# dart-icra/DART-Dual-Arm-Non-Prehensile-Manipulation

Measured on AMD Instinct MI355X. Metric: MPC solves/sec (horizon N=20, batch=18 objects) at 1/2/4/8 GPUs; max |u−u_ref|, higher is better.
Workload: dtype f64

## Files before the change

### dart-dual-arm-non-prehensile-manipulation_amd/csrc/pmpc_ipm.hip

```cpp
#if DART_WG == 2
#define dartmpc dartmpc_wg2
#endif
#include <hip/hip_runtime.h>
#include <stdint.h>
#include <stdlib.h>

#include "pmpc_ipm.h"
#include "pmpc_model.h"
#include "pmpc_resto.h"
#include "stamps.h"
#include "wave.h"

namespace dartmpc {

#ifdef DART_STAMPS
#ifndef PMPC_SEQ
__device__ unsigned long long g_stamp[32];
#define STAMP_FLUSH(b) STAMP_FLUSH32_TO(g_stamp, b)
#else
__device__ unsigned long long g_stamp_seq[32];
#define STAMP_FLUSH(b) STAMP_FLUSH32_TO(g_stamp_seq, b)
#endif
#else
#define STAMP_FLUSH(b) STAMP_FLUSH_TO(g_stamp, b)
// ... 119 lines not shown
    constexpr bool short2 = SHORT2 && !ONEROW;
    const double f11 = c.f11, a12k = c.a12k, a22k = c.a22k, ai12k = c.ai12k, ai22k = c.ai22k, a22i = c.a22i;
    const double uonf = c.uonf, A11k = c.A11k, A12k = c.A12k, A22k = c.A22k;
    (void)lane; (void)ai12k; (void)ai22k; (void)a22i; (void)uonf;
    const double X11d = lsm ? 1.0 : qp2 + delta, X22d = lsm ? 1.0 : qv2 + delta;
    double Quu[NAX], Rt[NAX];
#pragma unroll
    for (int j = 0; j < NAX; ++j) {
        P11[j] = X11d; P12[j] = 0.0; P22[j] = X22d;
        Rt[j] = (lsm ? 1.0 : Rt0[j]) + delta;
    }
    use_scan = false;
    if constexpr (NAX == 1 && QSCAN) {
        const double ratio = fmax(E11[0] * X11d, E22[0] * X22d);
        use_scan = !wany(uon && !(Rt[0] > 0.0 && ratio <= 2.0 * Rt[0]));
    }
    if (PM_EXPECT(use_scan, 1)) {
        const double iR = uon ? frcp(Rt[0]) : 0.0;
        const double G11 = be1[0] * be1[0] * iR, G12 = be1[0] * be2[0] * iR, G22 = be2[0] * be2[0] * iR;
        const double g11 = G11 + ai12k * G12, g12 = G12 + ai12k * G22, g21 = ai22k * G12, g22 = ai22k * G22;
        const double X11k = X11d * uonf, X22k = X22d * uonf;
        double T[16] = {1.0, ai12k, g11, g12,
                        0.0, ai22k, g21, g22,
                        X11k, X11k * ai12k, fma(X11k, g11, 1.0), X11k * g12,
                        0.0, X22k * ai22k, fma(X22k, g21, a12k), fma(X22k, g22, a22i)};
        mat4_scan_level<0x101, true>(T);
        mat4_scan_level<0x102>(T);
        mat4_scan_level<0x104>(T);
        if constexpr (!short2 && !one_row) mat4_scan_level<0x108>(T);
        double W[8] = {fma(T[2], X11d, T[0]), fma(T[3], X22d, T[1]), fma(T[6], X11d, T[4]),
                       fma(T[7], X22d, T[5]), fma(T[10], X11d, T[8]), fma(T[11], X22d, T[9]),
                       fma(T[14], X11d, T[12]), fma(T[15], X22d, T[13])};
        if constexpr (short2 || one_row) {
            double F[8];
            if constexpr (short2) {
#pragma unroll
            for (int e = 0; e < 8; ++e) F[e] = half_bcast_c<16>(W[e]);
            if ((lane & 16) == 0) {
#pragma unroll
                for (int i = 0; i < 4; ++i)
#pragma unroll
                    for (int jj = 0; jj < 2; ++jj)
                        W[2 * i + jj] = fma(T[4 * i], F[jj], fma(T[4 * i + 1], F[2 + jj],
                                            fma(T[4 * i + 2], F[4 + jj], T[4 * i + 3] * F[6 + jj])));
            }
            }
#pragma unroll
            for (int e = 0; e < 8; ++e) F[e] = dpp_fill<0x108, 0xf, 0>(W[e]);
            if ((lane & 24) == 0) {
#pragma unroll
                for (int i = 0; i < 4; ++i)
#pragma unroll
                    for (int jj = 0; jj < 2; ++jj)
                        W[2 * i + jj] = fma(T[4 * i], F[jj], fma(T[4 * i + 1], F[2 + jj],
                                            fma(T[4 * i + 2], F[4 + jj], T[4 * i + 3] * F[6 + jj])));
            }
        } else if constexpr (!one_row && kWaves == 1) {
            double F[8];
#pragma unroll
            for (int e = 0; e < 8; ++e) F[e] = half_bcast_c<16>(W[e]);
            if ((lane & 16) == 0) {
#pragma unroll
                for (int i = 0; i < 4; ++i)
#pragma unroll
                    for (int jj = 0; jj < 2; ++jj)
                        W[2 * i + jj] = fma(T[4 * i], F[jj], fma(T[4 * i + 1], F[2 + jj],
                                            fma(T[4 * i + 2], F[4 + jj], T[4 * i + 3] * F[6 + jj])));
            }
        }
        double pnx[3] = {0.0, 0.0, 0.0};
        if constexpr (kWaves == 2) {
            auto rows = [&]() {
                double F[8];
#pragma unroll
                for (int e = 0; e < 8; ++e) F[e] = half_bcast_c<16>(W[e]);
                if ((lane & 16) == 0) {
#pragma unroll
                    for (int i = 0; i < 4; ++i)
#pragma unroll
                        for (int jj = 0; jj < 2; ++jj)
                            W[2 * i + jj] = fma(T[4 * i], F[jj], fma(T[4 * i + 1], F[2 + jj],
                                                fma(T[4 * i + 2], F[4 + jj], T[4 * i + 3] * F[6 + jj])));
                }
            };
            double v[3] = {0.0, 0.0, 0.0}, pn[3];
            if (wave_idx() == 1) {
                rows();
                const double idet = frcp(fma(W[0], W[3], -W[1] * W[2]));
                v[0] = fma(W[4], W[3], -W[5] * W[2]) * idet;
                v[1] = 0.5 * (fma(W[5], W[0], -W[4] * W[1]) * idet + fma(W[6], W[3], -W[7] * W[2]) * idet);
                v[2] = fma(W[7], W[0], -W[6] * W[1]) * idet;
            }
            pm_pass<0>(1, 0, v, pn);
            pnx[0] = pn[0]; pnx[1] = pn[1]; pnx[2] = pn[2];
            if (wave_idx() == 0) {
#pragma unroll
                for (int i = 0; i < 4; ++i) {
                    W[2 * i] = fma(T[4 * i + 3], pn[1], fma(T[4 * i + 2], pn[0], T[4 * i]));
                    W[2 * i + 1] = fma(T[4 * i + 3], pn[2], fma(T[4 * i + 2], pn[1], T[4 * i + 1]));
                }
                rows();
            }
        }
        const double U11 = W[0], U12 = W[1], U21 = W[2], U22 = W[3];
        const double Y11 = W[4], Y12 = W[5], Y21 = W[6], Y22 = W[7];
        const double idet = frcp(fma(U11, U22, -U12 * U21));
        const double q11 = fma(Y11, U22, -Y12 * U21) * idet, q12 = fma(Y12, U11, -Y11 * U12) * idet;
        const double q21 = fma(Y21, U22, -Y22 * U21) * idet, q22 = fma(Y22, U11, -Y21 * U12) * idet;
        P11[0] = q11; P12[0] = 0.5 * (q12 + q21); P22[0] = q22;
        double n11, n12, n22;
        if constexpr (kWaves == 1) {
            n11 = from_next(P11[0]); n12 = from_next(P12[0]); n22 = from_next(P22[0]);
        } else {
            n11 = dpp<kWaveShl1>(P11[0]); n12 = dpp<kWaveShl1>(P12[0]); n22 = dpp<kWaveShl1>(P22[0]);
            if (wave_idx() == 0 && (lane & 31) == 31) { n11 = pnx[0]; n12 = pnx[1]; n22 = pnx[2]; }
        }
        const double e1 = be1[0], e2 = be2[0];
        const double Q = fma(E11[0], n11, fma(E12[0], n12, fma(E22[0], n22, Rt[0])));
        const double PB1 = fma(n11, e1, n12 * e2), PB2 = fma(n12, e1, n22 * e2);
        const double U1 = PB1, U2 = fma(PB1, a12k, PB2 * a22k);
        const double iQ = frcp(Q);
        W1[0] = iQ * U1; W2[0] = iQ * U2;
        Quu[0] = Q; iQs[0] = iQ;
    } else
    for (int step = 0; step < N; ++step) {
        double n11[NAX], n12[NAX], n22[NAX];
#pragma unroll
        for (int j = 0; j < NAX; ++j) {
            n11[j] = from_next(P11[j]); n12[j] = from_next(P12[j]); n22[j] = from_next(P22[j]);
        }
#pragma unroll
        for (int j = 0; j < NAX; ++j) {
            const double e1 = be1[j], e2 = be2[j];
            const double Q = fma(E11[j], n11[j], fma(E12[j], n12[j], fma(E22[j], n22[j], Rt[j])));
            const double PB1 = fma(n11[j], e1, n12[j] * e2), PB2 = fma(n12[j], e1, n22[j] * e2);
            const double U1 = PB1, U2 = fma(PB1, a12k, PB2 * a22k);
            const double X12 = fma(n11[j], a12k, n12[j] * a22k);
            const double X22 = fma(A11k, n11[j], fma(A12k, n12[j], fma(A22k, n22[j], X22d)));
            const double iQ = frcp(Q);
            const double w1 = iQ * U1, w2 = iQ * U2;
            P11[j] = fma(-w1, U1, fma(f11, n11[j], X11d));
            P12[j] = fma(-w1, U2, X12);
            P22[j] = fma(-w2, U2, X22);
            W1[j] = w1; W2[j] = w2;
            Quu[j] = Q; iQs[j] = iQ;
        }
    }
    bool bad = false;
#pragma unroll
    for (int j = 0; j < NAX; ++j) bad = bad || !(Quu[j] > 0.0) || !isfinite(Quu[j]);
    return !wany(bad);
}

enum PmPt { kPtTh, kPtSn, kPtLp, kPtLv, kPtZl, kPtZu, kPtP, kPtV, kPtZ, kPtMu, kPtRows };
enum PmFc { kFcP11, kFcP12, kFcP22, kFcW1, kFcW2, kFcIQs, kFcRows };
enum PmFlag { kFlStop, kFlUseScan, kFlOk, kFlFactorTime, kFlConverged, kFlMuDec, kFlEvalTime, kFlWords = 8 };
struct PmOvlShared {
    double pt[kPtRows][kWave];
    double fc[kFcRows][kWave];
    double mu_new;
    int flag[kFlWords];
};
__shared__ PmOvlShared g_pm_ovl;

__device__ __forceinline__ double pm_clamp_mult(const double z, const double mu, const double islack) {
    return fmax(fmin(z, 1e10 * mu * islack), 1e-10 * mu * islack);
}

enum : unsigned { kScan = 1u, kOneRow = 2u, kShort2 = 4u, kRed = 8u, kOcc2 = 16u, kFuse = 32u, kOvl = 64u };

template <int NAX, unsigned F>
__device__ __forceinline__ bool pmpc_solve(const PmpcArgs& a, const int b) {
    constexpr bool QSCAN = (F & kScan) != 0, ONEROW = (F & kOneRow) != 0, SHORT2 = (F & kShort2) != 0;
    constexpr bool RED = (F & kRed) != 0, OVL = (F & kOvl) != 0;
    static_assert(!OVL || (NAX == 1 && QSCAN && !ONEROW && !RED && kWaves == 1), "the overlapped build: scan builds of N = 16..31");
    STAMP_DECL
    const int lane = (kWaves == 1 && !OVL) ? (int)threadIdx.x : lane_id();
    const int k = NAX == 1 ? node_base() + (lane & 31) : lane;
    const int ax0 = NAX == 1 ? (lane >> 5) : 0;
    const int N = a.N;
    const bool xon = k <= N, uon = k < N;
    constexpr bool one_row = ONEROW;
    constexpr bool short2 = SHORT2 && !ONEROW;
    const double h = a.Ts;

    const double* st = a.x0 + 6 * b;
    const double* rf = a.ref + 6 * b;
    const double* pr = a.prm + 6 * b;
    const double mu_f = pr[0], Qp = pr[1], Qv = pr[2], R = pr[3], ulo = pr[4], uhi = pr[5];

    double a12, a22, b1, b2;
    axis_rk4(h, a.g, mu_f, 0.0, 0.0, 1.0, a12, a22);
    axis_rk4(h, a.g, mu_f, 1.0, 0.0, 0.0, b1, b2);
    double zp1, zav, zcp, zcv;
    z_rk4(h, 0.0, 1.0, 1.0, zp1, zav);
    z_rk4(h, 1.0, 0.0, 0.0, zcp, zcv);
    const double lo = ulo - 1e-8 * fmax(1.0, fabs(ulo));
    const double hi = uhi + 1e-8 * fmax(1.0, fabs(uhi));
    const bool poly = fmax(fabs(lo), fabs(hi)) <= 1.0;
    const double f11 = uon ? 1.0 : 0.0, a12k = uon ? a12 : 0.0, a22k = uon ? a22 : 0.0;
    const double ai22 = 1.0 / a22, ai12 = -a12 * ai22;
    const double uonf = uon ? 1.0 : 0.0, ai12k = uon ? ai12 : 0.0, ai22k = uon ? ai22 : 1.0, a22i = uon ? a22 : 1.0;
    const double A11k = a12k * a12k, A12k = 2.0 * a12k * a22k, A22k = a22k * a22k;

    double sp[NAX], sv[NAX], rp[NAX], rv[NAX];
    double p[NAX], v[NAX], th[NAX], lp[NAX], lv[NAX], zl[NAX], zu[NAX];
    double zA[NAX], zC[NAX], zs[NAX], zz[NAX];
    const int nw = 6 * (N + 1) + 2 * N;
    const double* ww = a.w_warm ? a.w_warm + (size_t)nw * b : nullptr;
    const double pushl = fmin(1e-2 * fmax(1.0, fabs(lo)), 1e-2 * (hi - lo));
    const double pushu = fmin(1e-2 * fmax(1.0, fabs(hi)), 1e-2 * (hi - lo));
    double gmax = 0.0;
#pragma unroll
    for (int j = 0; j < NAX; ++j) {
        const int ax = NAX == 1 ? ax0 : j;
        sp[j] = st[2 * ax]; sv[j] = st[2 * ax + 1];
        rp[j] = rf[2 * ax]; rv[j] = rf[2 * ax + 1];
        p[j] = xon ? (ww ? ww[6 * k + 2 * ax] : sp[j]) : 0.0;
        v[j] = xon ? (ww ? ww[6 * k + 2 * ax + 1] : sv[j]) : 0.0;
        double t = uon ? (ww ? ww[6 * (N + 1) + 2 * k + ax] : 0.0) : 0.0;
        if (uon) t = fmin(fmax(t, lo + pushl), hi - pushu);
        th[j] = t;
        lp[j] = 0.0; lv[j] = 0.0;
        zl[j] = uon ? 1.0 : 0.0; zu[j] = uon ? 1.0 : 0.0;
        if (xon) gmax = fmax(gmax, fmax(fabs(2 * Qp * (p[j] - rp[j])), fabs(2 * Qv * (v[j] - rv[j]))));
        if (uon) gmax = fmax(gmax, fabs(2 * R * th[j]));
        zA[j] = ax ? zav : zp1; zC[j] = ax ? zcv : zcp;
        zs[j] = st[4 + ax];
        zz[j] = xon ? (ww ? ww[6 * k + 4 + ax] : zs[j]) : 0.0;
    }
    gmax = wmax(gmax);
    const double sc = gmax > 100.0 ? 100.0 / gmax : 1.0;
    const double qp2 = sc * 2 * Qp, qv2 = sc * 2 * Qv, r2 = sc * 2 * R;
    const double scQp = sc * Qp, scQv = sc * Qv, scR = sc * R;
    const PmStage stg = {f11, a12k, a22k, ai12k, ai22k, a22i, uonf, A11k, A12k, A22k};
    auto quad_stage = [&](double csj, double snj, double lpnj, double lvnj, double zlj, double islj, double zuj,
                          double isuj, double& e1, double& e2, double& e11, double& e12, double& e22, double& rt0) {
        e1 = b1 * csj; e2 = b2 * csj;
        e11 = e1 * e1; e12 = 2.0 * e1 * e2; e22 = e2 * e2;
        rt0 = uon ? fma(snj, fma(b1, lpnj, b2 * lvnj), r2 + zlj * islj + zuj * isuj) : 1.0;
    };
    const double tol = a.tol, mu_min = tol / 10;
    const double n_eq = 6.0 * (N + 1), n_b = 4.0 * N;
    const double inv_neb = 1.0 / (n_eq + n_b), inv_nb = 1.0 / n_b;
    const double gam_th = 1e-5, gam_ph = 1e-8, s_th = 1.1, s_ph = 2.3, eta_ph = 1e-8, gam_al = 0.05;

    auto defects = [&](double pj, double vj, double sj, double spj, double svj, double& g1, double& g2) {
        const double fp = fma(a12, vj, fma(b1, sj, pj));
        const double fv = fma(a22, vj, b2 * sj);
        double ip, iv;
        if constexpr (kWaves == 1) {
            ip = from_prev(fp); iv = from_prev(fv);
        } else {
            const double x2[2] = {fp, fv};
            double o2[2];
            from_prev_n(x2, o2);
            ip = o2[0]; iv = o2[1];
        }
        g1 = (k == 0) ? pj - spj : pj - ip;
        g2 = (k == 0) ? vj - svj : vj - iv;
    };
    auto axes_sum = [&](const double (&q)[NAX]) -> double {
        if constexpr (NAX == 1) return half_pair_sum(q[0]);
        else return q[0] + q[1];
    };
    auto zdefect = [&](double zj, double wj, int j) -> double {
        const double fz = fma(zA[j], zj, zC[j] * wj);
        const double ip = from_prev(fz);
        return (k == 0) ? zj - zs[j] : zj - ip;
    };
    auto vz_new = [&](const double (&t)[NAX]) -> double {
        double sq[NAX];
#pragma unroll
        for (int j = 0; j < NAX; ++j) sq[j] = uon ? t[j] * t[j] : 0.0;
        return -a.g * axes_sum(sq);
    };

    auto point_verdict = [&](const double (&p)[NAX], const double (&v)[NAX], const double (&th)[NAX],
                             const double (&lp)[NAX], const double (&lv)[NAX], const double (&zl)[NAX],
                             const double (&zu)[NAX], const double (&g1)[NAX], const double (&g2)[NAX],
                             const double (&gz)[NAX], double& mu, bool& dec) -> bool {
        double dinf = 0.0, pinf = 0.0, c0 = 0.0, cmin = 1e300, suml = 0.0, sumz = 0.0;
#pragma unroll
        for (int j = 0; j < NAX; ++j) {
            const double c_ = tilt_cos_econ(poly, th[j]);
            const double cs = uon ? c_ : 0.0;
            const double ln = from_next(lp[j]), vn = from_next(lv[j]);
            const double lpn = uon ? ln : 0.0, lvn = uon ? vn : 0.0;
            const double sl = th[j] - lo, su = hi - th[j];
            const double r1 = fma(qp2, p[j] - rp[j], lp[j] - lpn);
            const double r2x = fma(qv2, v[j] - rv[j], lv[j] - fma(a12, lpn, a22 * lvn));
            const double ru = fma(r2, th[j], -cs * fma(b1, lpn, b2 * lvn)) - zl[j] + zu[j];
            dinf = fmax(dinf, xon ? fmax(fabs(r1), fabs(r2x)) : 0.0);
            dinf = fmax(dinf, uon ? fabs(ru) : 0.0);
            pinf = fmax(pinf, xon ? fmax(fmax(fabs(g1[j]), fabs(g2[j])), fabs(gz[j])) : 0.0);
            suml += xon ? fabs(lp[j]) + fabs(lv[j]) : 0.0;
            c0 = fmax(c0, uon ? fmax(zl[j] * sl, zu[j] * su) : 0.0);
            cmin = fmin(cmin, uon ? fmin(zl[j] * sl, zu[j] * su) : 1e300);
            sumz += zl[j] + zu[j];
        }
        float dinf_f = (float)dinf, pinf_f = (float)pinf, c0_f = (float)c0, cmin_f = (float)cmin;
        float suml_f = (float)suml, sumz_f = (float)sumz;
        wred_errors(dinf_f, pinf_f, c0_f, cmin_f, suml_f, sumz_f);
        const double dinf_w = dinf_f, pinf_w = pinf_f, c0_w = c0_f;
        const double cmin_w = cmin_f;
        const float sz_w = sumz_f;
        const double is_d = 100.0 * frcp(fmax(100.0, (double)(suml_f + sz_w) * inv_neb));
        const double is_c = 100.0 * frcp(fmax(100.0, (double)sz_w * inv_nb));
        dinf = dinf_w; pinf = pinf_w; c0 = c0_w;
        dec = false;
        if (fmax(dinf * is_d, fmax(pinf, c0 * is_c)) <= tol) return true;
        for (;;) {
            const double cmu = fmax(c0 - mu, mu - cmin_w);
            if (fmax(dinf * is_d, fmax(pinf, cmu * is_c)) > 10.0 * mu || mu <= mu_min) break;
            mu = fmax(mu_min, fmin(0.2 * mu, mu * sqrt(mu)));
            dec = true;
        }
        return false;
    };
    (void)point_verdict;
    if constexpr (OVL) {
        auto helper_rounds = [&](auto&& body) {
            const long long max_rounds = 2ll * a.max_iter + 8;
            for (long long round = 0; round < max_rounds; ++round) {
                __syncthreads();
                if (__builtin_amdgcn_readfirstlane(g_pm_ovl.flag[kFlStop])) return;
                body();
                __syncthreads();
                if (__builtin_amdgcn_readfirstlane(g_pm_ovl.flag[kFlStop])) return;
            }
        };
        const int wv = __builtin_amdgcn_readfirstlane((int)(threadIdx.x >> 6));
        if (wv == 1) {
            helper_rounds([&]() {
#ifdef DART_STAMPS
                const unsigned long long tf0 = __builtin_amdgcn_s_memtime();
#endif
                const double th1 = g_pm_ovl.pt[kPtTh][lane], sn1 = g_pm_ovl.pt[kPtSn][lane];
                const double lp1 = g_pm_ovl.pt[kPtLp][lane], lv1 = g_pm_ovl.pt[kPtLv][lane];
                const double zl1 = g_pm_ovl.pt[kPtZl][lane], zu1 = g_pm_ovl.pt[kPtZu][lane];
                const double c_ = tilt_cos_econ(poly, th1);
                const double cs1 = uon ? c_ : 0.0;
                const double ln = from_next(lp1), vn = from_next(lv1);
                const double lpn1 = uon ? ln : 0.0, lvn1 = uon ? vn : 0.0;
                const double sl = th1 - lo, su = hi - th1;
                const double isl1 = uon ? frcp(sl) : 0.0, isu1 = uon ? frcp(su) : 0.0;
                double be1[NAX], be2[NAX], E11[NAX], E12[NAX], E22[NAX], Rt0[NAX];
                quad_stage(cs1, sn1, lpn1, lvn1, zl1, isl1, zu1, isu1, be1[0], be2[0], E11[0], E12[0], E22[0], Rt0[0]);
                double W1[NAX], W2[NAX], P11[NAX], P12[NAX], P22[NAX], iQs[NAX];
                bool us = false;
                const bool okf = pmpc_riccati<NAX, QSCAN, ONEROW, SHORT2>(lane, N, uon, false, 0.0, qp2, qv2, stg, be1,
                                                                         be2, E11, E12, E22, Rt0, P11, P12, P22, W1,
                                                                         W2, iQs, us);
                g_pm_ovl.fc[kFcP11][lane] = P11[0]; g_pm_ovl.fc[kFcP12][lane] = P12[0]; g_pm_ovl.fc[kFcP22][lane] = P22[0];
                g_pm_ovl.fc[kFcW1][lane] = W1[0]; g_pm_ovl.fc[kFcW2][lane] = W2[0]; g_pm_ovl.fc[kFcIQs][lane] = iQs[0];
                if (lane == 0) { g_pm_ovl.flag[kFlUseScan] = us ? 1 : 0; g_pm_ovl.flag[kFlOk] = okf ? 1 : 0; }
#ifdef DART_STAMPS
                t_acc_[13] += __builtin_amdgcn_s_memtime() - tf0;
                if (lane == 0) g_pm_ovl.flag[kFlFactorTime] = (int)t_acc_[13];
#endif
            });
            return false;
        }
        if (wv == 2) {
            helper_rounds([&]() {
#ifdef DART_STAMPS
                const unsigned long long te0 = __builtin_amdgcn_s_memtime();
#endif
                const double th1[NAX] = {g_pm_ovl.pt[kPtTh][lane]}, sn1 = g_pm_ovl.pt[kPtSn][lane];
                const double lp1[NAX] = {g_pm_ovl.pt[kPtLp][lane]}, lv1[NAX] = {g_pm_ovl.pt[kPtLv][lane]};
                const double zl1[NAX] = {g_pm_ovl.pt[kPtZl][lane]}, zu1[NAX] = {g_pm_ovl.pt[kPtZu][lane]};
                const double p1[NAX] = {g_pm_ovl.pt[kPtP][lane]}, v1[NAX] = {g_pm_ovl.pt[kPtV][lane]};
                const double zz1 = g_pm_ovl.pt[kPtZ][lane];
                double mu1 = wave_uniform(g_pm_ovl.pt[kPtMu][lane]);
                double g1e[NAX], g2e[NAX], gze[NAX];
                const double w1 = vz_new(th1);
                defects(p1[0], v1[0], sn1, sp[0], sv[0], g1e[0], g2e[0]);
                gze[0] = zdefect(zz1, w1, 0);
                bool dec = false;
                const bool conv = point_verdict(p1, v1, th1, lp1, lv1, zl1, zu1, g1e, g2e, gze, mu1, dec);
                if (lane == 0) { g_pm_ovl.mu_new = mu1; g_pm_ovl.flag[kFlConverged] = conv ? 1 : 0; g_pm_ovl.flag[kFlMuDec] = dec ? 1 : 0; }
#ifdef DART_STAMPS
                t_acc_[17] += __builtin_amdgcn_s_memtime() - te0;
                if (lane == 0) g_pm_ovl.flag[kFlEvalTime] = (int)t_acc_[17];
#endif
            });
            return false;
        }
        if (lane == 0) g_pm_ovl.flag[kFlStop] = 0;
    }

    double g1[NAX], g2[NAX], gz[NAX], snc[NAX];
    double lgc[NAX];
    (void)lgc;
    double th0 = 0.0;
    {
        const double w0 = vz_new(th);
#pragma unroll
        for (int j = 0; j < NAX; ++j) {
            double s0, c0_;
            tilt_sincos(poly, th[j], s0, c0_);
            snc[j] = uon ? s0 : 0.0;
            if constexpr (OVL) lgc[j] = log_fast((th[j] - lo) * (hi - th[j]));
            defects(p[j], v[j], snc[j], sp[j], sv[j], g1[j], g2[j]);
            gz[j] = RED ? 0.0 : zdefect(zz[j], w0, j);
            if (xon) th0 += fabs(g1[j]) + fabs(g2[j]) + fabs(gz[j]);
        }
    }
    double theta = wsum(th0);
    const double th_max = 1e4 * fmax(1.0, theta), th_min = 1e-4 * fmax(1.0, theta);

    double fth = 0.0, fph = 0.0;
    int nfilt = 0;
    double mu = 0.1, delta_last = 0.0;
    int status = -1, it = 0;
    int in_soft = 0, soft_count = 0;
    STAMP(0);

    double zsm[4] = {0.0, 0.0, 0.0, 0.0};
    (void)zsm;
    if constexpr (OVL) {
        double m = k == 0 ? 0.0 : zA[0], c = 0.0;
        affine1_scan_level<0x111, 0xf>(m, c); zsm[0] = m;
        affine1_scan_level<0x112, 0xf>(m, c); zsm[1] = m;
        affine1_scan_level<0x114, 0xf>(m, c); zsm[2] = m;
        if constexpr (!short2) { affine1_scan_level<0x118, 0xf>(m, c); zsm[3] = m; }
    }

    bool published = false;
    auto publish = [&]() {
        __builtin_amdgcn_sched_barrier(0);
        g_pm_ovl.pt[kPtTh][lane] = th[0]; g_pm_ovl.pt[kPtSn][lane] = snc[0];
        g_pm_ovl.pt[kPtLp][lane] = lp[0]; g_pm_ovl.pt[kPtLv][lane] = lv[0];
        g_pm_ovl.pt[kPtZl][lane] = zl[0]; g_pm_ovl.pt[kPtZu][lane] = zu[0];
        g_pm_ovl.pt[kPtP][lane] = p[0]; g_pm_ovl.pt[kPtV][lane] = v[0];
        g_pm_ovl.pt[kPtZ][lane] = zz[0]; g_pm_ovl.pt[kPtMu][lane] = mu;
        __syncthreads();
        __builtin_amdgcn_sched_barrier(0);
        published = true;
    };
#ifdef DART_STAMPS
    const unsigned long long t_loop0 = __builtin_amdgcn_s_memtime();
#endif
    for (it = a.mult_init_max > 0.0 ? -1 : 0; it < a.max_iter; ++it) {
        const bool lsm = it < 0;
#ifdef DART_STAMPS
        if (it == 1) t_acc_[12] = __builtin_amdgcn_s_memtime() - t_loop0;
#endif
        if constexpr (OVL) {
            if (PM_EXPECT(!lsm && !published, 0)) publish();
        }
        double sn[NAX], cs[NAX], isl[NAX], isu[NAX], lpn[NAX], lvn[NAX];
        double dinf = 0.0, pinf = 0.0, c0 = 0.0, cmin = 1e300, suml = 0.0, sumz = 0.0;
#pragma unroll
        for (int j = 0; j < NAX; ++j) {
            sn[j] = snc[j];
            const double c_ = tilt_cos_econ(poly, th[j]);
            cs[j] = uon ? c_ : 0.0;
            double ln, vn;
            if constexpr (kWaves == 1) {
                ln = from_next(lp[j]); vn = from_next(lv[j]);
            } else {
                const double x2[2] = {lp[j], lv[j]};
                double o2[2];
                from_next_n(x2, o2);
                ln = o2[0]; vn = o2[1];
            }
            lpn[j] = uon ? ln : 0.0; lvn[j] = uon ? vn : 0.0;
            const double sl = th[j] - lo, su = hi - th[j];
            isl[j] = uon ? frcp(sl) : 0.0; isu[j] = uon ? frcp(su) : 0.0;
            STAMP(16);
            const double r1 = fma(qp2, p[j] - rp[j], lp[j] - lpn[j]);
            const double r2x = fma(qv2, v[j] - rv[j], lv[j] - fma(a12, lpn[j], a22 * lvn[j]));
            const double ru = fma(r2, th[j], -cs[j] * fma(b1, lpn[j], b2 * lvn[j])) - zl[j] + zu[j];
            if constexpr (!OVL) {
            dinf = fmax(dinf, xon ? fmax(fabs(r1), fabs(r2x)) : 0.0);
            dinf = fmax(dinf, uon ? fabs(ru) : 0.0);
            pinf = fmax(pinf, xon ? fmax(fmax(fabs(g1[j]), fabs(g2[j])), fabs(gz[j])) : 0.0);
            suml += xon ? fabs(lp[j]) + fabs(lv[j]) : 0.0;
            c0 = fmax(c0, uon ? fmax(zl[j] * sl, zu[j] * su) : 0.0);
            cmin = fmin(cmin, uon ? fmin(zl[j] * sl, zu[j] * su) : 1e300);
            sumz += zl[j] + zu[j];
            }
        }
        float dinf_f = (float)dinf, pinf_f = (float)pinf, c0_f = (float)c0, cmin_f = (float)cmin;
        float suml_f = (float)suml, sumz_f = (float)sumz;
        if constexpr (!OVL) wred_errors(dinf_f, pinf_f, c0_f, cmin_f, suml_f, sumz_f);
        const double dinf_w = dinf_f, pinf_w = pinf_f, c0_w = c0_f;
        const double cmin_w = cmin_f;
        const float sz_w = sumz_f;
        const double is_d = 100.0 * frcp(fmax(100.0, (double)(suml_f + sz_w) * inv_neb));
        const double is_c = 100.0 * frcp(fmax(100.0, (double)sz_w * inv_nb));
        dinf = dinf_w; pinf = pinf_w; c0 = c0_w;
        STAMP(1);
        if constexpr (!OVL) {
        if (!lsm && fmax(dinf * is_d, fmax(pinf, c0 * is_c)) <= tol) { status = 0; break; }
        }
        if constexpr (!OVL) {
        for (; !lsm;) {
            const double cmu = fmax(c0 - mu, mu - cmin_w);
            if (fmax(dinf * is_d, fmax(pinf, cmu * is_c)) > 10.0 * mu || mu <= mu_min) break;
            mu = fmax(mu_min, fmin(0.2 * mu, mu * sqrt(mu)));
            nfilt = 0; in_soft = 0;
        }
        }
        double tau = fmax(0.99, 1.0 - mu);
        STAMP(2);

        double be1[NAX], be2[NAX], E11[NAX], E12[NAX], E22[NAX], Rt0[NAX], rt[NAX], q1[NAX], q2[NAX];
#pragma unroll
        for (int j = 0; j < NAX; ++j) {
            quad_stage(cs[j], sn[j], lpn[j], lvn[j], zl[j], isl[j], zu[j], isu[j], be1[j], be2[j], E11[j], E12[j],
                       E22[j], Rt0[j]);
            if (!OVL || lsm) rt[j] = uon ? (lsm ? r2 * th[j] - zl[j] + zu[j] : fma(r2, th[j], mu * (isu[j] - isl[j]))) : 0.0;
            q1[j] = qp2 * (p[j] - rp[j]); q2[j] = qv2 * (v[j] - rv[j]);
        }
        double W1[NAX], W2[NAX], P11[NAX], P12[NAX], P22[NAX], iQs[NAX];
        double delta = 0.0;
        bool ok = false;
        int attempt = 0;
        if constexpr (OVL) {
            if (!lsm) {
                __builtin_amdgcn_sched_barrier(0);
                SPAN_BEGIN(t_b);
                __syncthreads();
                SPAN_END(14, t_b);
                const int usf = g_pm_ovl.flag[kFlUseScan], okff = g_pm_ovl.flag[kFlOk];
                const int cvf = g_pm_ovl.flag[kFlConverged], mdf = g_pm_ovl.flag[kFlMuDec];
                const double mun = g_pm_ovl.mu_new;
                P11[0] = g_pm_ovl.fc[kFcP11][lane]; P12[0] = g_pm_ovl.fc[kFcP12][lane]; P22[0] = g_pm_ovl.fc[kFcP22][lane];
                W1[0] = g_pm_ovl.fc[kFcW1][lane]; W2[0] = g_pm_ovl.fc[kFcW2][lane]; iQs[0] = g_pm_ovl.fc[kFcIQs][lane];
                const bool us = __builtin_amdgcn_readfirstlane(usf) != 0;
                const bool okf = __builtin_amdgcn_readfirstlane(okff) != 0;
                if (__builtin_amdgcn_readfirstlane(cvf)) { status = 0; break; }
                mu = wave_uniform(mun);
                if (__builtin_amdgcn_readfirstlane(mdf)) { nfilt = 0; in_soft = 0; }
                tau = fmax(0.99, 1.0 - mu);
                rt[0] = uon ? fma(r2, th[0], mu * (isu[0] - isl[0])) : 0.0;
                if (PM_EXPECT(us && okf, 1)) {
                    STAMP_ADD(11, 1);
                    ok = true; attempt = 1;
                }
            }
        }
        for (; attempt < 60 && !ok; ++attempt) {
            if (PM_EXPECT(attempt > 0, 0))
                delta = (attempt == 1) ? (delta_last == 0.0 ? 1e-4 : fmax(1e-20, delta_last * (1.0 / 3.0)))
                                       : delta * (delta_last == 0.0 ? 100.0 : 8.0);
            bool use_scan = false;
            ok = pmpc_riccati<NAX, QSCAN, ONEROW, SHORT2>(lane, N, uon, lsm, delta, qp2, qv2, stg, be1, be2, E11, E12,
                                                          E22, Rt0, P11, P12, P22, W1, W2, iQs, use_scan);
            STAMP_ADD(11, use_scan ? 1 : 0);
        }
        STAMP_ADD(9, attempt);
        STAMP(3);
        if (PM_EXPECT(!ok, 0)) { status = -3; break; }
        if (delta > 0.0) delta_last = delta;

        double dp[NAX], dv[NAX], dth[NAX], dlp[NAX], dlv[NAX], dzl[NAX], dzu[NAX], dz[NAX];
        double amax = 1.0, az = 1.0;
        float am_lf = 1.0f, az_lf = 1.0f;
        const double (&g1o)[NAX] = g1, (&g2o)[NAX] = g2, (&gzo)[NAX] = gz;
        auto direction = [&]() {
            double p1[NAX], p2[NAX], kff[NAX], gn1[NAX], gn2[NAX], g1[NAX], g2[NAX], gz[NAX];
#pragma unroll
            for (int j = 0; j < NAX; ++j) {
                g1[j] = lsm ? 0.0 : g1o[j]; g2[j] = lsm ? 0.0 : g2o[j]; gz[j] = lsm ? 0.0 : gzo[j];
            }
            double nPw[3];
            if constexpr (kWaves == 1) {
#pragma unroll
                for (int j = 0; j < NAX; ++j) { gn1[j] = from_next(g1[j]); gn2[j] = from_next(g2[j]); }
            } else {
                const double x5[5] = {g1[0], g2[0], P11[0], P12[0], P22[0]};
                double o5[5];
                from_next_n(x5, o5);
                gn1[0] = o5[0]; gn2[0] = o5[1]; nPw[0] = o5[2]; nPw[1] = o5[3]; nPw[2] = o5[4];
            }
            if constexpr (NAX == 1) {
                const double e1 = be1[0], e2 = be2[0], w1 = W1[0], w2 = W2[0];
                const double nP11 = kWaves == 1 ? from_next(P11[0]) : nPw[0];
                const double nP12 = kWaves == 1 ? from_next(P12[0]) : nPw[1];
                const double nP22 = kWaves == 1 ? from_next(P22[0]) : nPw[2];
                const double t1 = fma(nP11, gn1[0], nP12 * gn2[0]), t2 = fma(nP12, gn1[0], nP22 * gn2[0]);
                double m11 = fma(-w1, e1, f11), m12 = -w1 * e2, m21 = fma(-w2, e1, a12k), m22 = fma(-w2, e2, a22k);
// ... 57 lines not shown
                    if (wave_idx() == 0 && (lane & 31) == 31) { np1 = p32[0]; np2 = p32[1]; }
                }
                const double h1 = np1 - t1, h2 = np2 - t2;
                kff[0] = -iQs[0] * fma(e1, h1, fma(e2, h2, rtk));

                double pw1, pw2, pkf, pb1, pb2;
                if constexpr (kWaves == 1) {
                    pw1 = from_prev(W1[0]); pw2 = from_prev(W2[0]); pkf = from_prev(kff[0]);
                    pb1 = from_prev(be1[0]); pb2 = from_prev(be2[0]);
                } else {
                    const double x5[5] = {W1[0], W2[0], kff[0], be1[0], be2[0]};
                    double o5[5];
                    from_prev_n(x5, o5);
                    pw1 = o5[0]; pw2 = o5[1]; pkf = o5[2]; pb1 = o5[3]; pb2 = o5[4];
                }
                double f11_ = 1.0 - pb1 * pw1, f12_ = fma(-pb1, pw2, a12), f21_ = -pb2 * pw1, f22_ = fma(-pb2, pw2, a22);
                double d1 = fma(pb1, pkf, -g1[0]), d2 = fma(pb2, pkf, -g2[0]);
                if (k == 0) { f11_ = 0.0; f12_ = 0.0; f21_ = 0.0; f22_ = 0.0; d1 = -g1[0]; d2 = -g2[0]; }
                affine_scan_level<0x111, 0xf>(f11_, f12_, f21_, f22_, d1, d2);
                affine_scan_level<0x112, 0xf>(f11_, f12_, f21_, f22_, d1, d2);
                affine_scan_level<0x114, 0xf>(f11_, f12_, f21_, f22_, d1, d2);
                if constexpr (one_row || short2) affine_scan_const<0x118, 0xf>(f11_, f12_, f21_, f22_, d1, d2);
                else affine_scan_level<0x118, 0xf>(f11_, f12_, f21_, f22_, d1, d2);
                if constexpr (kWaves == 1) {
                    if constexpr (!one_row) affine_scan_const<0x142, 0xa>(f11_, f12_, f21_, f22_, d1, d2);
                } else {
                    if (wave_idx() == 0) affine_scan_const<0x142, 0xa>(f11_, f12_, f21_, f22_, d1, d2);
                    double r[2];
                    { const double v[2] = {d1, d2}; pm_pass<2>(0, 31, v, r); }
                    if (wave_idx() == 1) {
                        if ((lane & 16) == 0) {
                            d1 = fma(f11_, r[0], fma(f12_, r[1], d1));
                            d2 = fma(f21_, r[0], fma(f22_, r[1], d2));
                        }
                        affine_scan_const<0x142, 0xa>(f11_, f12_, f21_, f22_, d1, d2);
                    }
                }
                dp[0] = d1; dv[0] = d2;
            } else {
                double nP11[NAX], nP12[NAX], nP22[NAX];
#pragma unroll
                for (int j = 0; j < NAX; ++j) {
                    nP11[j] = from_next(P11[j]); nP12[j] = from_next(P12[j]); nP22[j] = from_next(P22[j]);
                    p1[j] = q1[j]; p2[j] = q2[j]; kff[j] = 0.0;
                }
                for (int step = 0; step < N; ++step) {
                    double n1[NAX], n2[NAX];
#pragma unroll
                    for (int j = 0; j < NAX; ++j) { n1[j] = from_next(p1[j]); n2[j] = from_next(p2[j]); }
#pragma unroll
                    for (int j = 0; j < NAX; ++j) {
                        const double h1 = n1[j] - fma(nP11[j], gn1[j], nP12[j] * gn2[j]);
                        const double h2 = n2[j] - fma(nP12[j], gn1[j], nP22[j] * gn2[j]);
                        const double qu = fma(be1[j], h1, fma(be2[j], h2, rt[j]));
                        kff[j] = -iQs[j] * qu;
                        p1[j] = fma(-W1[j], qu, fma(f11, h1, q1[j]));
                        p2[j] = fma(-W2[j], qu, q2[j] + fma(a12k, h1, a22k * h2));
                    }
                }
#pragma unroll
                for (int j = 0; j < NAX; ++j) { dp[j] = -g1[j]; dv[j] = -g2[j]; }
                for (int step = 0; step < N; ++step) {
                    double op[NAX], ov[NAX];
#pragma unroll
                    for (int j = 0; j < NAX; ++j) {
                        const double dt_ = fma(-W1[j], dp[j], fma(-W2[j], dv[j], kff[j]));
                        op[j] = fma(a12, dv[j], fma(be1[j], dt_, dp[j]));
                        ov[j] = fma(a22, dv[j], be2[j] * dt_);
                    }
#pragma unroll
                    for (int j = 0; j < NAX; ++j) {
                        const double ip = from_prev(op[j]), iv = from_prev(ov[j]);
                        dp[j] = k >= 1 ? ip - g1[j] : dp[j];
                        dv[j] = k >= 1 ? iv - g2[j] : dv[j];
                    }
                }
            }
            double am = 1.0, az_ = 1.0, twd[NAX];
#pragma unroll
            for (int j = 0; j < NAX; ++j) {
                dth[j] = uon ? fma(-W1[j], dp[j], fma(-W2[j], dv[j], kff[j])) : 0.0;
                dlp[j] = xon ? -fma(P11[j], dp[j], fma(P12[j], dv[j], p1[j])) - lp[j] : 0.0;
                dlv[j] = xon ? -fma(P12[j], dp[j], fma(P22[j], dv[j], p2[j])) - lv[j] : 0.0;
                const double sl = th[j] - lo, su = hi - th[j];
                const double zlx = zl[j] * isl[j], zux = zu[j] * isu[j];
                dzl[j] = uon ? fma(-zlx, dth[j], fma(mu, isl[j], -zl[j])) : 0.0;
                dzu[j] = uon ? fma(zux, dth[j], fma(mu, isu[j], -zu[j])) : 0.0;
                const double ith = frcp(dth[j]);
                const double cand = dth[j] < 0 ? -tau * sl * ith : (dth[j] > 0 ? tau * su * ith : 1.0);
                const double czl = dzl[j] < 0 ? -tau * zl[j] * frcp(dzl[j]) : 1.0;
                const double czu = dzu[j] < 0 ? -tau * zu[j] * frcp(dzu[j]) : 1.0;
                am = fmin(am, uon ? cand : 1.0);
                az_ = fmin(az_, uon ? fmin(czl, czu) : 1.0);
                twd[j] = 2.0 * th[j] * dth[j];
            }
            am_lf = (float)am; az_lf = (float)az_;
            const double wd = RED ? 0.0 : -a.g * axes_sum(twd);
            if constexpr (RED) {
#pragma unroll
                for (int j = 0; j < NAX; ++j) dz[j] = 0.0;
            } else if constexpr (NAX == 1) {
                const double src = from_prev(zC[0] * wd);
                double m = k == 0 ? 0.0 : zA[0], c = k == 0 ? -gz[0] : src - gz[0];
                if constexpr (OVL) {
                    affine1_scan_const<0x111, 0xf>(m, c);
                    affine1_scan_const<0x112, 0xf>(zsm[0], c);
                    affine1_scan_const<0x114, 0xf>(zsm[1], c);
                    affine1_scan_const<0x118, 0xf>(zsm[2], c);
                    m = short2 ? zsm[2] : zsm[3];
                } else {
                affine1_scan_level<0x111, 0xf>(m, c);
                affine1_scan_level<0x112, 0xf>(m, c);
                affine1_scan_level<0x114, 0xf>(m, c);
                if constexpr (one_row || short2) affine1_scan_const<0x118, 0xf>(m, c);
                else affine1_scan_level<0x118, 0xf>(m, c);
                }
                if constexpr (kWaves == 1) {
                    if constexpr (!one_row) affine1_scan_const<0x142, 0xa>(m, c);
                } else {
                    if (wave_idx() == 0) affine1_scan_const<0x142, 0xa>(m, c);
                    double r[1];
                    { const double v[1] = {c}; pm_pass<3>(0, 31, v, r); }
                    if (wave_idx() == 1) {
                        if ((lane & 16) == 0) c = fma(m, r[0], c);
                        affine1_scan_const<0x142, 0xa>(m, c);
                    }
                }
                dz[0] = c;
            } else {
#pragma unroll
                for (int j = 0; j < NAX; ++j) dz[j] = -gz[j];
                for (int step = 0; step < N; ++step) {
#pragma unroll
                    for (int j = 0; j < NAX; ++j) {
                        const double ip = from_prev(fma(zA[j], dz[j], zC[j] * wd));
                        dz[j] = k >= 1 ? ip - gz[j] : dz[j];
                    }
                }
            }
        };

        auto frac_set = [&]() {
            amax = (double)am_lf * (1.0 - 1.0 / 1048576.0);
            az = (double)az_lf * (1.0 - 1.0 / 1048576.0);
        };

        double alpha = 1.0, amain = 1.0, th_t = 0.0, ph_t = 0.0, th_old = 0.0, phi = 0.0, gTd = 0.0, amin = 0.0;
        float lg_sw = 0.0f;
        bool accepted = false, ftype = false, tiny = false;
        int ls = 0, soc = 0;
        double snt[NAX], g1t[NAX], g2t[NAX], gzt[NAX];
        double lgt[NAX];
        (void)lgt;
        double sn_pre = 0.0;
        bool sn_pre_on = false;
        (void)sn_pre; (void)sn_pre_on;
        auto trial = [&](double al) {
            double thl = 0.0, phl = 0.0, tt[NAX];
            if constexpr (kWaves == 2 && NAX == 1 && !RED) {
                const double pt = fma(al, dp[0], p[0]), vt = fma(al, dv[0], v[0]);
                tt[0] = fma(al, dth[0], th[0]);
                double s_, c_;
                tilt_sincos(poly, tt[0], s_, c_);
                snt[0] = uon ? s_ : 0.0;
                const double wt = vz_new(tt);
                const double zt = fma(al, dz[0], zz[0]);
                const double x3[3] = {fma(a12, vt, fma(b1, snt[0], pt)), fma(a22, vt, b2 * snt[0]),
                                      fma(zA[0], zt, zC[0] * wt)};
                double o3[3];
                from_prev_n(x3, o3);
                g1t[0] = (k == 0) ? pt - sp[0] : pt - o3[0];
                g2t[0] = (k == 0) ? vt - sv[0] : vt - o3[1];
                gzt[0] = (k == 0) ? zt - zs[0] : zt - o3[2];
                const double ep = pt - rp[0], ev = vt - rv[0];
                thl += xon ? fabs(g1t[0]) + fabs(g2t[0]) : 0.0;
                phl += xon ? fma(scQp * ep, ep, scQv * ev * ev) : 0.0;
                phl += uon ? fma(scR * tt[0], tt[0], -mu * log_fast((tt[0] - lo) * (hi - tt[0]))) : 0.0;
                thl += xon ? fabs(gzt[0]) : 0.0;
                wsum2(thl, phl);
                th_t = thl; ph_t = phl;
                return;
            }
#pragma unroll
            for (int j = 0; j < NAX; ++j) {
                const double pt = fma(al, dp[j], p[j]), vt = fma(al, dv[j], v[j]);
                tt[j] = fma(al, dth[j], th[j]);
                if (OVL && PM_EXPECT(sn_pre_on, 1)) {
                    snt[j] = sn_pre; sn_pre_on = false;
                } else {
                    double s_, c_;
                    tilt_sincos(poly, tt[j], s_, c_);
                    snt[j] = uon ? s_ : 0.0;
                }
                defects(pt, vt, snt[j], sp[j], sv[j], g1t[j], g2t[j]);
                const double ep = pt - rp[j], ev = vt - rv[j];
                thl += xon ? fabs(g1t[j]) + fabs(g2t[j]) : 0.0;
                phl += xon ? fma(scQp * ep, ep, scQv * ev * ev) : 0.0;
                if constexpr (OVL) {
                    lgt[j] = log_fast((tt[j] - lo) * (hi - tt[j]));
                    phl += uon ? fma(scR * tt[j], tt[j], -mu * lgt[j]) : 0.0;
                } else {
                    phl += uon ? fma(scR * tt[j], tt[j], -mu * log_fast((tt[j] - lo) * (hi - tt[j]))) : 0.0;
                }
            }
            if constexpr (RED) {
#pragma unroll
                for (int j = 0; j < NAX; ++j) gzt[j] = 0.0;
            } else {
                const double wt = vz_new(tt);
#pragma unroll
                for (int j = 0; j < NAX; ++j) {
                    gzt[j] = zdefect(fma(al, dz[j], zz[j]), wt, j);
                    thl += xon ? fabs(gzt[j]) : 0.0;
                }
            }
            wsum2(thl, phl);
            th_t = thl; ph_t = phl;
        };
        auto acceptable = [&](double al_test, bool& ft) {
            bool in_filter = !(th_t < th_max) || !isfinite(ph_t);
            in_filter = in_filter || wany_rep(lane < nfilt && th_t >= fth && ph_t >= fph);
            if (in_filter) return false;
            const bool sw = gTd < 0.0 && lg2(al_test) > lg_sw;
            if (theta <= th_min && sw) {
                if (cmp_le(ph_t, phi + eta_ph * al_test * gTd, phi)) { ft = true; return true; }
                return false;
            }
            return cmp_le(th_t, (1 - gam_th) * theta, theta) || cmp_le(ph_t - phi, -gam_ph * theta, phi);
        };
        if (PM_EXPECT(lsm, 0)) {
            direction();
            double ym = 0.0;
#pragma unroll
            for (int j = 0; j < NAX; ++j) ym = fmax(ym, xon ? fmax(fabs(dlp[j]), fabs(dlv[j])) : 0.0);
            if (wmax(ym) <= a.mult_init_max) {
#pragma unroll
                for (int j = 0; j < NAX; ++j) { lp[j] += dlp[j]; lv[j] += dlv[j]; }
            }
            continue;
        }
        for (;;) {
            direction();
            if (PM_EXPECT(soc != 0, 0)) { wmin2f(am_lf, az_lf); frac_set(); }
            STAMP(4);
            if (PM_EXPECT(soc == 0, 1)) {
                double phil = 0.0, gtdl = 0.0;
#pragma unroll
                for (int j = 0; j < NAX; ++j) {
                    const double ep = p[j] - rp[j], ev = v[j] - rv[j];
                    const double sl = th[j] - lo, su = hi - th[j];
                    phil += xon ? fma(scQp * ep, ep, scQv * ev * ev) : 0.0;
                    gtdl += xon ? fma(qp2 * ep, dp[j], qv2 * ev * dv[j]) : 0.0;
                    if constexpr (OVL) phil += uon ? fma(scR * th[j], th[j], -mu * lgc[j]) : 0.0;
                    else phil += uon ? fma(scR * th[j], th[j], -mu * log_fast(sl * su)) : 0.0;
                    gtdl += uon ? rt[j] * dth[j] : 0.0;
                }
                float tn_w = 0.0f;
#pragma unroll
                for (int j = 0; j < NAX; ++j) {
                    tn_w = fmaxf(tn_w, xon ? fabsf((float)dp[j]) * __builtin_amdgcn_rcpf(1.0f + fabsf((float)p[j])) : 0.0f);
                    tn_w = fmaxf(tn_w, xon ? fabsf((float)dv[j]) * __builtin_amdgcn_rcpf(1.0f + fabsf((float)v[j])) : 0.0f);
                    tn_w = fmaxf(tn_w, xon ? fabsf((float)dz[j]) * __builtin_amdgcn_rcpf(1.0f + fabsf((float)zz[j])) : 0.0f);
                    tn_w = fmaxf(tn_w, uon ? fabsf((float)dth[j]) * __builtin_amdgcn_rcpf(1.0f + fabsf((float)th[j])) : 0.0f);
                }
                wsum2_maxf_min2f(phil, gtdl, tn_w, am_lf, az_lf);
                frac_set();
                phi = phil; gTd = gtdl;
                const float lg_th = theta > 0.0 ? lg2(theta) : -3.0e38f;
                const float lg_gd = gTd < 0.0 ? lg2(-gTd) : 3.0e38f;
                lg_sw = (float)s_th * lg_th - (float)s_ph * lg_gd;
                amin = gam_th;
                if (gTd < 0.0) amin = fmin(gam_th, fmin(gam_ph * theta * frcp(-gTd), (double)__builtin_amdgcn_exp2f(fmaxf(lg_sw, -126.0f))));
                amin *= gam_al;
                tiny = tn_w < 2.2e-15f;
                alpha = amax; amain = amax;
                if constexpr (OVL) {
                    const double thc = fma(alpha, dth[0], th[0]);
                    double s_, c_;
                    tilt_sincos(poly, thc, s_, c_);
                    sn_pre = uon ? s_ : 0.0; sn_pre_on = true;
                    const double il = frcp(thc - lo), iu = frcp(hi - thc);
                    const double zln = pm_clamp_mult(fma(az, dzl[0], zl[0]), mu, il);
                    const double zun = pm_clamp_mult(fma(az, dzu[0], zu[0]), mu, iu);
                    __builtin_amdgcn_sched_barrier(0);
                    g_pm_ovl.pt[kPtTh][lane] = thc; g_pm_ovl.pt[kPtSn][lane] = sn_pre;
                    g_pm_ovl.pt[kPtLp][lane] = fma(alpha, dlp[0], lp[0]); g_pm_ovl.pt[kPtLv][lane] = fma(alpha, dlv[0], lv[0]);
                    g_pm_ovl.pt[kPtZl][lane] = uon ? zln : 0.0; g_pm_ovl.pt[kPtZu][lane] = uon ? zun : 0.0;
                    g_pm_ovl.pt[kPtP][lane] = fma(alpha, dp[0], p[0]); g_pm_ovl.pt[kPtV][lane] = fma(alpha, dv[0], v[0]);
                    g_pm_ovl.pt[kPtZ][lane] = fma(alpha, dz[0], zz[0]); g_pm_ovl.pt[kPtMu][lane] = mu;
                    __syncthreads();
                    __builtin_amdgcn_sched_barrier(0);
                }
            } else if (soc > 0) {
                alpha = amax;
            }
            STAMP(5);
            bool again = false;
            if constexpr ((NAX == 2 || kWaves == 2) && !RED) {
                if (PM_EXPECT(in_soft, 0)) break;
                if (PM_EXPECT(soc < 0 && alpha < amin, 0)) break;
            }
            for (;;) {
                trial(alpha);
                bool ft = false;
                if (PM_EXPECT(soc == 0 && tiny, 0)) { accepted = true; ftype = true; break; }
                if (acceptable(soc > 0 ? amain : alpha, ft)) { accepted = true; ftype = ft; break; }
                if (PM_EXPECT(!RED && soc == 0 && ls == 0 && a.max_soc > 0 && !(th_t < theta), 0)) {
#pragma unroll
                    for (int j = 0; j < NAX; ++j) {
                        g1[j] = fma(alpha, g1[j], g1t[j]); g2[j] = fma(alpha, g2[j], g2t[j]);
                        gz[j] = fma(alpha, gz[j], gzt[j]);
                    }
                    th_old = th_t; soc = 1; again = true;
                    break;
                }
                if (PM_EXPECT(soc > 0, 0)) {
                    if (soc < a.max_soc && th_t <= 0.99 * th_old) {
#pragma unroll
                        for (int j = 0; j < NAX; ++j) {
                            g1[j] = fma(alpha, g1[j], g1t[j]); g2[j] = fma(alpha, g2[j], g2t[j]);
                            gz[j] = fma(alpha, gz[j], gzt[j]);
                        }
                        th_old = th_t; ++soc; again = true;
                        break;
                    }
                    const double w0 = RED ? 0.0 : vz_new(th);
#pragma unroll
                    for (int j = 0; j < NAX; ++j) {
                        defects(p[j], v[j], snc[j], sp[j], sv[j], g1[j], g2[j]);
                        gz[j] = RED ? 0.0 : zdefect(zz[j], w0, j);
                    }
                    soc = -1; ls = 1; alpha = 0.5 * amain;
                    again = ((NAX == 2 || kWaves == 2) && !RED) || !(alpha < amin);
                    break;
                }
                ++ls;
                alpha *= 0.5;
                if (alpha < amin || ls >= 80) break;
            }
            if (!again) break;
        }
        STAMP_ADD(10, ls + 1);
        STAMP_ADD(15, soc > 0 ? 1 : 0);
        STAMP(6);
        bool soft = false;
        if (PM_EXPECT(!accepted, 0)) {
            if constexpr (!RED && (NAX == 2 || kWaves == 2)) {
                if (a.soft) {
                    if (!in_soft) {
                        if (nfilt < kWave) {
                            if (lane == nfilt) { fth = (1 - gam_th) * theta; fph = phi - gam_ph * theta; }
                            ++nfilt;
                        }
                        soft_count = 0;
                    }
                    if (!(in_soft && ++soft_count > 10)) {
                        double am = 1.0, a2 = 1.0;
#pragma unroll
                        for (int j = 0; j < NAX; ++j) {
                            if (uon) {
                                const double sl = th[j] - lo, su = hi - th[j];
                                if (dth[j] < 0) am = fmin(am, -tau * sl / dth[j]);
                                if (dth[j] > 0) am = fmin(am, tau * su / dth[j]);
                                if (dzl[j] < 0) a2 = fmin(a2, -tau * zl[j] / dzl[j]);
                                if (dzu[j] < 0) a2 = fmin(a2, -tau * zu[j] / dzu[j]);
                            }
                        }
                        const double as = fmin(wmin(am), wmin(a2));
                        trial(as);
                        bool ft_ = false;
                        const bool orig = acceptable(0.0, ft_);
                        bool take = orig;
                        if (!take && isfinite(ph_t)) {
                            double pd[2];
#pragma unroll 1
                            for (int pass = 0; pass < 2; ++pass) {
                                const double sa = pass ? as : 0.0;
                                double t = 0.0;
#pragma unroll
                                for (int j = 0; j < NAX; ++j) {
                                    const double pp = fma(sa, dp[j], p[j]), vv = fma(sa, dv[j], v[j]);
                                    const double tt = fma(sa, dth[j], th[j]);
                                    const double lpv = fma(sa, dlp[j], lp[j]), lvv = fma(sa, dlv[j], lv[j]);
                                    const double zlv = uon ? fma(sa, dzl[j], zl[j]) : 0.0;
                                    const double zuv = uon ? fma(sa, dzu[j], zu[j]) : 0.0;
                                    const double ga = pass ? g1t[j] : g1[j], gb = pass ? g2t[j] : g2[j];
                                    const double gc = pass ? gzt[j] : gz[j];
                                    const double ln = from_next(lpv), vn = from_next(lvv);
                                    const double lpn_ = uon ? ln : 0.0, lvn_ = uon ? vn : 0.0;
                                    const double r1 = fma(qp2, pp - rp[j], lpv - lpn_);
                                    const double r2x = fma(qv2, vv - rv[j], lvv - fma(a12, lpn_, a22 * lvn_));
                                    const double c_ = tilt_cos_econ(poly, tt);
                                    const double ru = fma(r2, tt, -c_ * fma(b1, lpn_, b2 * lvn_)) - zlv + zuv;
                                    const double sl = tt - lo, su = hi - tt;
                                    t += xon ? fabs(r1) + fabs(r2x) + fabs(ga) + fabs(gb) + fabs(gc) : 0.0;
                                    t += uon ? fabs(ru) + fabs(zlv * sl - mu) + fabs(zuv * su - mu) : 0.0;
                                }
                                pd[pass] = wsum(t);
                            }
                            take = pd[1] <= 0.9999 * pd[0];
                        }
                        if (take) {
                            accepted = true; soft = true; alpha = as; az = as;
                            in_soft = orig ? 0 : 1;
                            if (orig) soft_count = 0;
                        }
                    }
                }
            }
            if (!accepted) { status = a.resto ? kPmNeedResto : -2; break; }
        }
        if (!soft && !ftype && nfilt < kWave) {
            if (lane == nfilt) { fth = (1 - gam_th) * theta; fph = phi - gam_ph * theta; }
            ++nfilt;
        }
        const bool hit = OVL && soc == 0 && ls == 0;
        if constexpr (OVL) {
            STAMP_ADD(15, hit ? (1ull << 16) : (1ull << 32));
            if (PM_EXPECT(!hit, 0)) {
                __builtin_amdgcn_sched_barrier(0);
                __syncthreads();
                __builtin_amdgcn_sched_barrier(0);
            }
        }
#pragma unroll
        for (int j = 0; j < NAX; ++j) {
            snc[j] = snt[j];
            lp[j] = fma(alpha, dlp[j], lp[j]); lv[j] = fma(alpha, dlv[j], lv[j]);
            th[j] = fma(alpha, dth[j], th[j]);
            if (OVL && PM_EXPECT(hit, 1)) {
                zl[j] = g_pm_ovl.pt[kPtZl][lane]; zu[j] = g_pm_ovl.pt[kPtZu][lane];
            } else {
                const double il = frcp(th[j] - lo), iu = frcp(hi - th[j]);
                const double zln = pm_clamp_mult(fma(az, dzl[j], zl[j]), mu, il);
                const double zun = pm_clamp_mult(fma(az, dzu[j], zu[j]), mu, iu);
                zl[j] = uon ? zln : 0.0; zu[j] = uon ? zun : 0.0;
            }
        }
        if constexpr (OVL) {
            p[0] = fma(alpha, dp[0], p[0]); v[0] = fma(alpha, dv[0], v[0]);
            zz[0] = fma(alpha, dz[0], zz[0]);
            if (PM_EXPECT(!hit, 0)) publish();
        }
#pragma unroll
        for (int j = 0; j < NAX; ++j) {
// ... 347 lines not shown
```

Before: 342,600.

## Publish speculative trial point earlier and let helper waves compute sine themselves

In the overlapped multi-wave IPM path, the main wave now publishes the speculative full-step trial point to shared memory right after the fraction-to-boundary reduction. Before, it published only after the merit and directional-derivative reductions. The sine of the tilt angle is no longer precomputed and shared: each helper wave (factorization and evaluation) recomputes it, and the main wave's trial recomputes it too. The intent is to start the helper waves' speculative work sooner and shorten the main wave's critical path, at the cost of some duplicated transcendental work and a split of the fused reduction into two.

```diff
diff --git a/dart-dual-arm-non-prehensile-manipulation_amd/csrc/pmpc_ipm.hip b/dart-dual-arm-non-prehensile-manipulation_amd/csrc/pmpc_ipm.hip
--- a/dart-dual-arm-non-prehensile-manipulation_amd/csrc/pmpc_ipm.hip
+++ b/dart-dual-arm-non-prehensile-manipulation_amd/csrc/pmpc_ipm.hip
@@ -295,7 +295,7 @@
     return !wany(bad);
 }
 
-enum PmPt { kPtTh, kPtSn, kPtLp, kPtLv, kPtZl, kPtZu, kPtP, kPtV, kPtZ, kPtMu, kPtRows };
+enum PmPt { kPtTh, kPtLp, kPtLv, kPtZl, kPtZu, kPtP, kPtV, kPtZ, kPtMu, kPtRows };
 enum PmFc { kFcP11, kFcP12, kFcP22, kFcW1, kFcW2, kFcIQs, kFcRows };
 enum PmFlag { kFlStop, kFlUseScan, kFlOk, kFlFactorTime, kFlConverged, kFlMuDec, kFlEvalTime, kFlWords = 8 };
 struct PmOvlShared {
@@ -479,9 +479,12 @@
 #ifdef DART_STAMPS
                 const unsigned long long tf0 = __builtin_amdgcn_s_memtime();
 #endif
-                const double th1 = g_pm_ovl.pt[kPtTh][lane], sn1 = g_pm_ovl.pt[kPtSn][lane];
+                const double th1 = g_pm_ovl.pt[kPtTh][lane];
                 const double lp1 = g_pm_ovl.pt[kPtLp][lane], lv1 = g_pm_ovl.pt[kPtLv][lane];
                 const double zl1 = g_pm_ovl.pt[kPtZl][lane], zu1 = g_pm_ovl.pt[kPtZu][lane];
+                double s_, sc_;
+                tilt_sincos(poly, th1, s_, sc_);
+                const double sn1 = uon ? s_ : 0.0;
                 const double c_ = tilt_cos_econ(poly, th1);
                 const double cs1 = uon ? c_ : 0.0;
                 const double ln = from_next(lp1), vn = from_next(lv1);
@@ -510,7 +513,7 @@
 #ifdef DART_STAMPS
                 const unsigned long long te0 = __builtin_amdgcn_s_memtime();
 #endif
-                const double th1[NAX] = {g_pm_ovl.pt[kPtTh][lane]}, sn1 = g_pm_ovl.pt[kPtSn][lane];
+                const double th1[NAX] = {g_pm_ovl.pt[kPtTh][lane]};
                 const double lp1[NAX] = {g_pm_ovl.pt[kPtLp][lane]}, lv1[NAX] = {g_pm_ovl.pt[kPtLv][lane]};
                 const double zl1[NAX] = {g_pm_ovl.pt[kPtZl][lane]}, zu1[NAX] = {g_pm_ovl.pt[kPtZu][lane]};
                 const double p1[NAX] = {g_pm_ovl.pt[kPtP][lane]}, v1[NAX] = {g_pm_ovl.pt[kPtV][lane]};
@@ -518,6 +521,9 @@
                 double mu1 = wave_uniform(g_pm_ovl.pt[kPtMu][lane]);
                 double g1e[NAX], g2e[NAX], gze[NAX];
                 const double w1 = vz_new(th1);
+                double s_, sc_;
+                tilt_sincos(poly, th1[0], s_, sc_);
+                const double sn1 = uon ? s_ : 0.0;
                 defects(p1[0], v1[0], sn1, sp[0], sv[0], g1e[0], g2e[0]);
                 gze[0] = zdefect(zz1, w1, 0);
                 bool dec = false;
@@ -573,7 +579,7 @@
     bool published = false;
     auto publish = [&]() {
         __builtin_amdgcn_sched_barrier(0);
-        g_pm_ovl.pt[kPtTh][lane] = th[0]; g_pm_ovl.pt[kPtSn][lane] = snc[0];
+        g_pm_ovl.pt[kPtTh][lane] = th[0];
         g_pm_ovl.pt[kPtLp][lane] = lp[0]; g_pm_ovl.pt[kPtLv][lane] = lv[0];
         g_pm_ovl.pt[kPtZl][lane] = zl[0]; g_pm_ovl.pt[kPtZu][lane] = zu[0];
         g_pm_ovl.pt[kPtP][lane] = p[0]; g_pm_ovl.pt[kPtV][lane] = v[0];
@@ -937,9 +943,6 @@
         double snt[NAX], g1t[NAX], g2t[NAX], gzt[NAX];
         double lgt[NAX];
         (void)lgt;
-        double sn_pre = 0.0;
-        bool sn_pre_on = false;
-        (void)sn_pre; (void)sn_pre_on;
         auto trial = [&](double al) {
             double thl = 0.0, phl = 0.0, tt[NAX];
             if constexpr (kWaves == 2 && NAX == 1 && !RED) {
@@ -970,13 +973,9 @@
             for (int j = 0; j < NAX; ++j) {
                 const double pt = fma(al, dp[j], p[j]), vt = fma(al, dv[j], v[j]);
                 tt[j] = fma(al, dth[j], th[j]);
-                if (OVL && PM_EXPECT(sn_pre_on, 1)) {
-                    snt[j] = sn_pre; sn_pre_on = false;
-                } else {
-                    double s_, c_;
-                    tilt_sincos(poly, tt[j], s_, c_);
-                    snt[j] = uon ? s_ : 0.0;
-                }
+                double s_, c_;
+                tilt_sincos(poly, tt[j], s_, c_);
+                snt[j] = uon ? s_ : 0.0;
                 defects(pt, vt, snt[j], sp[j], sv[j], g1t[j], g2t[j]);
                 const double ep = pt - rp[j], ev = vt - rv[j];
                 thl += xon ? fabs(g1t[j]) + fabs(g2t[j]) : 0.0;
@@ -1029,6 +1028,23 @@
             if (PM_EXPECT(soc != 0, 0)) { wmin2f(am_lf, az_lf); frac_set(); }
             STAMP(4);
             if (PM_EXPECT(soc == 0, 1)) {
+                if constexpr (OVL) {
+                    wmin2f(am_lf, az_lf);
+                    frac_set();
+                    alpha = amax; amain = amax;
+                    const double thc = fma(alpha, dth[0], th[0]);
+                    const double il = frcp(thc - lo), iu = frcp(hi - thc);
+                    const double zln = pm_clamp_mult(fma(az, dzl[0], zl[0]), mu, il);
+                    const double zun = pm_clamp_mult(fma(az, dzu[0], zu[0]), mu, iu);
+                    __builtin_amdgcn_sched_barrier(0);
+                    g_pm_ovl.pt[kPtTh][lane] = thc;
+                    g_pm_ovl.pt[kPtLp][lane] = fma(alpha, dlp[0], lp[0]); g_pm_ovl.pt[kPtLv][lane] = fma(alpha, dlv[0], lv[0]);
+                    g_pm_ovl.pt[kPtZl][lane] = uon ? zln : 0.0; g_pm_ovl.pt[kPtZu][lane] = uon ? zun : 0.0;
+                    g_pm_ovl.pt[kPtP][lane] = fma(alpha, dp[0], p[0]); g_pm_ovl.pt[kPtV][lane] = fma(alpha, dv[0], v[0]);
+                    g_pm_ovl.pt[kPtZ][lane] = fma(alpha, dz[0], zz[0]); g_pm_ovl.pt[kPtMu][lane] = mu;
+                    __syncthreads();
+                    __builtin_amdgcn_sched_barrier(0);
+                }
                 double phil = 0.0, gtdl = 0.0;
 #pragma unroll
                 for (int j = 0; j < NAX; ++j) {
@@ -1048,8 +1064,11 @@
                     tn_w = fmaxf(tn_w, xon ? fabsf((float)dz[j]) * __builtin_amdgcn_rcpf(1.0f + fabsf((float)zz[j])) : 0.0f);
                     tn_w = fmaxf(tn_w, uon ? fabsf((float)dth[j]) * __builtin_amdgcn_rcpf(1.0f + fabsf((float)th[j])) : 0.0f);
                 }
+                if constexpr (OVL) wsum2_maxf(phil, gtdl, tn_w);
+                else {
                 wsum2_maxf_min2f(phil, gtdl, tn_w, am_lf, az_lf);
                 frac_set();
+                }
                 phi = phil; gTd = gtdl;
                 const float lg_th = theta > 0.0 ? lg2(theta) : -3.0e38f;
                 const float lg_gd = gTd < 0.0 ? lg2(-gTd) : 3.0e38f;
@@ -1059,23 +1078,6 @@
                 amin *= gam_al;
                 tiny = tn_w < 2.2e-15f;
                 alpha = amax; amain = amax;
-                if constexpr (OVL) {
-                    const double thc = fma(alpha, dth[0], th[0]);
-                    double s_, c_;
-                    tilt_sincos(poly, thc, s_, c_);
-                    sn_pre = uon ? s_ : 0.0; sn_pre_on = true;
-                    const double il = frcp(thc - lo), iu = frcp(hi - thc);
-                    const double zln = pm_clamp_mult(fma(az, dzl[0], zl[0]), mu, il);
-                    const double zun = pm_clamp_mult(fma(az, dzu[0], zu[0]), mu, iu);
-                    __builtin_amdgcn_sched_barrier(0);
-                    g_pm_ovl.pt[kPtTh][lane] = thc; g_pm_ovl.pt[kPtSn][lane] = sn_pre;
-                    g_pm_ovl.pt[kPtLp][lane] = fma(alpha, dlp[0], lp[0]); g_pm_ovl.pt[kPtLv][lane] = fma(alpha, dlv[0], lv[0]);
-                    g_pm_ovl.pt[kPtZl][lane] = uon ? zln : 0.0; g_pm_ovl.pt[kPtZu][lane] = uon ? zun : 0.0;
-                    g_pm_ovl.pt[kPtP][lane] = fma(alpha, dp[0], p[0]); g_pm_ovl.pt[kPtV][lane] = fma(alpha, dv[0], v[0]);
-                    g_pm_ovl.pt[kPtZ][lane] = fma(alpha, dz[0], zz[0]); g_pm_ovl.pt[kPtMu][lane] = mu;
-                    __syncthreads();
-                    __builtin_amdgcn_sched_barrier(0);
-                }
             } else if (soc > 0) {
                 alpha = amax;
             }
```

After: 360,800, median of 6. +5.3%, better.
